# Christopher-Wang/DistriFlow

Measured on AMD Instinct MI355X. Metric: images/sec (whole node), MNIST CNN sync-SGD at 1/2/4/8 MI355X; async speedup, higher is better.
Workload: dtype bf16; 1 GPU; model=lenet5, global_batch=4096, per_gpu_batch=4096, parallelism=dp1, optimizer=sgd, graph=full, steps_per_graph=64, p2p_reason=single rank, step=train+reduce/update, params=61706

## Files before the change

csrc/bindings_fused.cpp:

```cpp
#include "bindings_comm.h"

namespace dfa_py {
namespace {

struct CPIn {
  const void* x = nullptr;
  int u8 = 0;
  const long long* idx = nullptr;
  long long nrows = 0;
};

CPIn cp_input(const torch::Tensor& x, const c10::optional<torch::Tensor>& idx, int64_t B, int64_t HWC) {
  CPIn r;
  TORCH_CHECK(x.is_cuda() && x.is_contiguous(), "x must be a contiguous GPU tensor");
  if (has(idx)) {
    need(*idx, at::kLong, "idx");
    TORCH_CHECK(idx->numel() >= B, "idx shorter than the batch");
    TORCH_CHECK(x.scalar_type() == at::kByte || x.scalar_type() == at::kBFloat16, "dataset must be u8 or bf16");
    TORCH_CHECK(x.dim() >= 1 && x.size(0) > 0 && x.numel() / x.size(0) == HWC, "dataset row size mismatch");
    TORCH_CHECK(x.scalar_type() == at::kByte, "indexed input must be a uint8 dataset");
    r.u8 = 1;
    r.idx = reinterpret_cast<const long long*>(idx->data_ptr<int64_t>());
    r.nrows = x.size(0);
  } else {
// ... 294 lines not shown

void lenet_train_py(torch::Tensor x, c10::optional<torch::Tensor> idx, double scale, torch::Tensor labels,
                    std::vector<torch::Tensor> conv, std::vector<torch::Tensor> dense_w,
                    std::vector<torch::Tensor> dense_wt, std::vector<torch::Tensor> dense_b,
                    std::vector<torch::Tensor> conv_grads, std::vector<torch::Tensor> dense_gw,
                    std::vector<torch::Tensor> dense_gb, std::vector<torch::Tensor> hT, std::vector<torch::Tensor> dzT,
                    torch::Tensor conv_part, torch::Tensor dense_part, torch::Tensor loss_part, torch::Tensor stats,
                    torch::Tensor frag, torch::Tensor ftab, torch::Tensor pxtab, int64_t B, double grad_scale,
                    bool prep, c10::optional<torch::Tensor> snap, std::vector<torch::Tensor> conv_mom,
                    c10::optional<torch::Tensor> sgd_master, c10::optional<torch::Tensor> sgd_mom,
                    c10::optional<torch::Tensor> sgd_wbf, c10::optional<torch::Tensor> sgd_hyper,
                    c10::optional<torch::Tensor> sgd_descs, c10::optional<torch::Tensor> idx_stream,
                    c10::optional<torch::Tensor> idx_cursor, c10::optional<torch::Tensor> idx_dst,
                    const P2PComm* ll, int64_t exch_blocks, c10::optional<torch::Tensor> run_stats,
                    const PSComm* ps, c10::optional<torch::Tensor> ps_perm, c10::optional<torch::Tensor> ps_idx,
                    double ps_lr, int64_t ps_max_stale, bool red_succ) {
  TORCH_CHECK(conv.size() == 4 && conv_grads.size() == 4, "lenet: conv = [w1, b1, w2, b2]");
  TORCH_CHECK(dense_w.size() == 3 && dense_wt.size() == 3 && dense_b.size() == 3 && dense_gw.size() == 3 &&
                  dense_gb.size() == 3 && hT.size() == 3 && dzT.size() == 3,
              "lenet: three dense layers");
  TORCH_CHECK(B > 0 && B < (1 << 30), "lenet: bad batch");
  dfa::LeNetArgs a{};
  const int64_t ldt = (B + 31) / 32 * 32;
  const int64_t lds = hT.size() == 3 && hT[0].dim() == 2 ? hT[0].size(1) : 0;
  TORCH_CHECK(lds >= ldt && lds % 32 == 0, "lenet: hT rows must hold round32(B) columns, stride a multiple of 32");
  if (x.scalar_type() == at::kByte) {
    TORCH_CHECK(x.is_cuda() && x.is_contiguous() && x.numel() % 784 == 0, "lenet: uint8 dataset [N][28][28][1]");
    a.x_u8 = x.data_ptr<uint8_t>();
    a.nrows = x.numel() / 784;
    TORCH_CHECK(has(idx) || a.nrows >= B,
                "lenet: a uint8 dataset without batch indices must hold the batch (rows 0 .. B-1)");
// ... 63 lines not shown
  a.loss_part = loss_part.data_ptr<float>();
  auto bp = [](torch::Tensor& t) { return reinterpret_cast<dfa::bf16*>(t.data_ptr()); };
  a.h0T = bp(hT[0]); a.h1T = bp(hT[1]); a.h2T = bp(hT[2]);
  a.dz1T = bp(dzT[0]); a.dz2T = bp(dzT[1]); a.dz3T = bp(dzT[2]);
  TORCH_CHECK(frag.is_cuda() && frag.is_contiguous() && (size_t)frag.nbytes() >= dfa::lenet_frag_bytes(),
              "lenet: fragment buffer too small");
  TORCH_CHECK(ftab.is_cuda() && ftab.scalar_type() == at::kByte && ftab.numel() == 98 * 2 * 16, "lenet: ftab");
  TORCH_CHECK(pxtab.is_cuda() && pxtab.scalar_type() == at::kShort && pxtab.numel() == 832, "lenet: pxtab");
  a.frag = frag.data_ptr();
  a.prep = prep ? 1 : 0;
  a.ftab = ftab.data_ptr<uint8_t>();
  a.pxtab = reinterpret_cast<const unsigned short*>(pxtab.data_ptr());
  a.B = (int)B;
  a.ldt = (int)lds;
  a.grad_scale = (float)grad_scale;
  dfa::LeNetRedArgs r{};
  r.kcols = (int)ldt;
  need(dense_part, at::kFloat, "lenet dense_part");
  TORCH_CHECK(dense_part.numel() >= dfa::lenet_dense_part_floats((int)B),
              "lenet: dense_part must hold lenet_dense_part_floats(B) zero-initialised floats");
  dfa::lenet_red_bind_scratch(dense_part.data_ptr<float>(), r);
  r.succ = red_succ ? 1 : 0;
  r.conv_part = a.conv_part;
  r.loss_part = a.loss_part;
  r.stats = stats.data_ptr<float>();
  r.g_w1 = conv_grads[0].data_ptr<float>();
  r.g_b1 = conv_grads[1].data_ptr<float>();
  r.g_w2 = conv_grads[2].data_ptr<float>();
  r.g_b2 = conv_grads[3].data_ptr<float>();
  for (int l = 0; l < 3; ++l) {
// ... 220 lines not shown
        py::arg("x"), py::arg("idx"), py::arg("scale"), py::arg("B"), py::arg("w1"), py::arg("b1"), py::arg("kpad1"),
        py::arg("w2t"), py::arg("dyp"), py::arg("code"), py::arg("slabs"), py::arg("g_w1"), py::arg("g_b1"),
        py::arg("g_w2"), py::arg("g_b2"), py::arg("step_inc") = py::none());
  m.def("kcnn_slab_floats", [](int64_t B) { return (int64_t)dfa::kcnn_slab_floats((int)B); });
  m.def("lenet_train", &lenet_train_py, "whole-network LeNet-5 training step (fwd + CE + bwd, 2 launches)",
        py::arg("x"), py::arg("idx"), py::arg("scale"), py::arg("labels"), py::arg("conv"), py::arg("dense_w"),
        py::arg("dense_wt"), py::arg("dense_b"), py::arg("conv_grads"), py::arg("dense_gw"), py::arg("dense_gb"),
        py::arg("hT"), py::arg("dzT"), py::arg("conv_part"), py::arg("dense_part"), py::arg("loss_part"),
        py::arg("stats"), py::arg("frag"), py::arg("ftab"), py::arg("pxtab"), py::arg("B"), py::arg("grad_scale"),
        py::arg("prep") = true, py::arg("snap") = py::none(),
        py::arg("conv_mom") = std::vector<torch::Tensor>{}, py::arg("sgd_master") = py::none(),
        py::arg("sgd_mom") = py::none(), py::arg("sgd_wbf") = py::none(), py::arg("sgd_hyper") = py::none(),
        py::arg("sgd_descs") = py::none(), py::arg("idx_stream") = py::none(), py::arg("idx_cursor") = py::none(),
        py::arg("idx_dst") = py::none(), py::arg("ll") = nullptr, py::arg("exch_blocks") = 0, py::arg("run_stats") = py::none(),
        py::arg("ps") = nullptr, py::arg("ps_perm") = py::none(), py::arg("ps_idx") = py::none(),
        py::arg("ps_lr") = 0.0, py::arg("ps_max_stale") = -1, py::arg("red_succ") = true);
  m.def("lenet_blocks", [](int64_t B) { return dfa::lenet_blocks((int)B); });
  m.def("lenet_frag_bytes", []() { return (int64_t)dfa::lenet_frag_bytes(); });
  m.def("lenet_dense_part_floats", [](int64_t B) { return (int64_t)dfa::lenet_dense_part_floats((int)B); });
  m.def("lenet_red_err_offset", []() { return (int64_t)dfa::lenet_red_err_offset(); });
}

void bind_comm(py::module_& m) {
  py::class_<P2PComm>(m, "P2PComm", "one-shot xGMI all-reduce over IPC-mapped peer buffers")
      .def(py::init<int64_t, int64_t, int64_t, double, int64_t>(), py::arg("rank"), py::arg("world"),
           py::arg("max_floats"), py::arg("timeout_s") = 2.0, py::arg("ll_slots") = 256)
      .def("handle", &P2PComm::handle)
      .def("open", &P2PComm::open)
      .def("allreduce", &P2PComm::allreduce, py::arg("t"), py::arg("scale") = 1.0)
      .def("error", &P2PComm::error)
      .def("host_error", &P2PComm::host_error)
      .def("ll_selftest", &P2PComm::ll_selftest, py::arg("inp"), py::arg("out"))
// ... 56 lines not shown
```

csrc/kernels.h:

```cpp
#pragma once
#include <hip/hip_runtime_api.h>
#include <stddef.h>
#include <stdint.h>

#include "ps_layout.h"

namespace dfa {
typedef __bf16 bf16;
}

namespace dfa {

enum { MODE_DIRECT = 0, MODE_FWD = 1, MODE_DGRAD = 2 };

struct DropSpec {
  int on;
  unsigned thresh;
  float p, scale;
  unsigned long long seed;
  const long long* step;
  int step_add;
};
inline DropSpec make_drop(float p, unsigned long long seed, const long long* step, int step_add = 0) {
  DropSpec d{};
// ... 398 lines not shown
  float* conv_part;
  float* loss_part;
  bf16 *h0T, *h1T, *h2T;
  bf16 *dz1T, *dz2T, *dz3T;
  float* logits;
  int prep;
  const void* frag;
  const unsigned char* ftab;
  const unsigned short* pxtab;
  unsigned long long* stamps;
  int B, ldt;
  float grad_scale;
  int nblk, ps_admit;
  int ps_excl;
  int ipw;
  PSArgs ps;
};
struct LeNetDense {
  const bf16* dzT;
  const bf16* hT;
  float* gw;
  float* gb;
  int N, K, tiles;
};
struct LeNetSgd {
  float* master;
  float* mom;
  bf16* wbf;
  const float* hyper;
  ParamDesc d[10];
// ... 106 lines not shown
  int ldt, jobs, nloss;
  const float* loss_part;
  float* stats;
};
hipError_t khead_wgrad(KHeadWgradArgs a, hipStream_t st);
size_t khead_ws_floats(int B, int K);
size_t khead_err_offset(int B);
size_t khead_lds(int K);
bool khead_supported(int K, int C);
hipError_t khead_train(KHeadArgs a, hipStream_t st);
int lenet_dense_part_floats(int B);
void lenet_red_bind_scratch(float* dense_part, LeNetRedArgs& r);
int lenet_red_err_offset();
size_t lenet_train_lds();
int lenet_blocks(int B);
hipError_t lenet_train(const LeNetArgs& a, LeNetRedArgs r, hipStream_t st);
void lenet_set_stamps(void* buf);
size_t lenet_frag_bytes();

enum MetricKind {
  kMetricMSE = 0, kMetricAbs = 1, kMetricHinge = 2, kMetricHuber = 3, kMetricLog = 4, kMetricSigmoidCE = 5,
  kMetricSoftmaxCE = 6, kMetricCategoricalCE = 7
};
hipError_t classifier_metrics(const float* z, const int* labels, int B, int C, int kind, int softmax, float* out,
                              hipStream_t st);

enum ActKind {
  kActLinear = 0, kActRelu = 1, kActRelu6 = 2, kActSigmoid = 3, kActTanh = 4, kActElu = 5, kActSelu = 6,
  kActSoftplus = 7, kActSoftsign = 8, kActHardSigmoid = 9, kActSwish = 10, kActExp = 11
};
// ... 36 lines not shown
```

csrc/lenet_fused.hip:

```cpp
#include "common.h"
#include "diag.h"
#include "kernels.h"
#include "lenet_frag.h"
#include "ll_exchange.h"
#include "optim_device.h"
#include "ps_device.h"

#include <algorithm>
#include <cstdlib>
#include <vector>

namespace dfa {
namespace {

constexpr int IMG = 8;
constexpr int NT = 512;
constexpr int NW = NT / 64;
constexpr int ccdiv(int a, int b) { return (a + b - 1) / b; }
constexpr int XS_ELEMS = IMG * 1024 + 32;
constexpr int OFF_XS = 0;
constexpr int OFF_P1 = OFF_XS + XS_ELEMS * 2;
constexpr int OFF_C1 = OFF_P1 + IMG * 196 * 16;
constexpr int DC2_RS = 104;
constexpr int NM = IMG * DC2_RS;
// ... 26 lines not shown
constexpr int LDS_BYTES = OFF_ST + 128;
static_assert(OFF_U == OFF_C1 + IMG * 196 * 4 + 128 + 98 * 2 * 16 + 800 * 2 + 128 && OFF_U % 16 == 0 && OFF_KZ % 16 == 0 && OFF_H1 % 16 == 0 && OFF_ZR % 16 == 0 && OFF_C2 % 16 == 0 && OFF_RED % 16 == 0 && OFF_DB % 16 == 0 && OFF_ST % 16 == 0 &&
                  OFF_PX % 16 == 0 && OFF_W % 16 == 0,
              "LDS carve must stay 16-byte aligned");
static_assert(2 * LDS_BYTES <= 160 * 1024, "two workgroups per CU");

typedef __bf16 bf16x4_vs __attribute__((__vector_size__(8)));

#define LN_STAMP(slot)                                                            \
  do {                                                                            \
    if (stamps) {                                                                 \
      __builtin_amdgcn_sched_barrier(0);                                          \
      unsigned long long t_;                                                      \
      asm volatile("s_memtime %0\n\ts_waitcnt lgkmcnt(0)" : "=s"(t_)::"memory"); \
      __builtin_amdgcn_sched_barrier(0);                                          \
      if (threadIdx.x == 0) STMP[(slot)] = t_;                                    \
    }                                                                             \
  } while (0)

template <int CTRL>
__device__ __forceinline__ float dpp_f(float v) {
  return __builtin_bit_cast(float, __builtin_amdgcn_update_dpp(0, __builtin_bit_cast(int, v), CTRL, 0xf, 0xf, false));
}
__device__ __forceinline__ float row16_max(float v) {
  v = fmaxf(v, dpp_f<0xB1>(v));
  v = fmaxf(v, dpp_f<0x4E>(v));
  v = fmaxf(v, dpp_f<0x141>(v));
  return fmaxf(v, dpp_f<0x140>(v));
}
__device__ __forceinline__ float row16_sum(float v) {
  v += dpp_f<0xB1>(v);
// ... 14 lines not shown
  for (int e = 0; e < 4; ++e) {
    r[e] = a[e];
    r[e + 4] = b[e];
  }
  return r;
}
__device__ __forceinline__ bf16x8 ld8(const bf16* p) { return *reinterpret_cast<const bf16x8*>(p); }
__device__ __forceinline__ void st8(bf16* p, const bf16x8& v) { *reinterpret_cast<bf16x8*>(p) = v; }
__device__ __forceinline__ bf16x8 zero8() {
  bf16x8 z;
#pragma unroll
  for (int e = 0; e < 8; ++e) z[e] = (bf16)0.f;
  return z;
}

__device__ __forceinline__ void build_shift1(const bf16* Xs, bf16* Xs1) {
  for (int t = threadIdx.x; t < XS_ELEMS / 8 - 1; t += NT) {
    const uint4 lo = *reinterpret_cast<const uint4*>(Xs + 8 * t);
    const unsigned nx = *reinterpret_cast<const unsigned*>(Xs + 8 * t + 8);
    uint4 o;
    o.x = __builtin_amdgcn_alignbyte(lo.y, lo.x, 2);
    o.y = __builtin_amdgcn_alignbyte(lo.z, lo.y, 2);
    o.z = __builtin_amdgcn_alignbyte(lo.w, lo.z, 2);
    o.w = __builtin_amdgcn_alignbyte(nx, lo.w, 2);
    *reinterpret_cast<uint4*>(Xs1 + 8 * t) = o;
  }
}

__device__ __forceinline__ void pool4(float a00, float a01, float a10, float a11, float& best, unsigned& code) {
  best = a00;
  code = 0;
  if (a01 > best) { best = a01; code = 1; }
  if (a10 > best) { best = a10; code = 2; }
  if (a11 > best) { best = a11; code = 3; }
  if (!(best > 0.f)) { best = 0.f; code = 4; }
}

template <int KS, int NTW>
struct DenseFrags {
  bf16x8 b[NTW][KS];
};
template <int KS, int NTW>
__device__ __forceinline__ void dense_load(DenseFrags<KS, NTW>& f, const bf16* __restrict__ W, int ntiles) {
  const int lane = threadIdx.x & 63, w = threadIdx.x >> 6, i = lane & 15, g = lane >> 4;
#pragma unroll
  for (int tt = 0; tt < NTW; ++tt) {
    const int t = w + NW * tt;
    if (t < ntiles) {
      const bf16* wrow = W + (long long)(16 * t + i) * (32 * KS) + 8 * g;
#pragma unroll
      for (int s = 0; s < KS; ++s) f.b[tt][s] = ld8(wrow + 32 * s);
    }
  }
}

template <int KS, int NTW>
__device__ __forceinline__ void dense_fwd(const DenseFrags<KS, NTW>& f, const bf16* A, int lda, const bf16* zr,
                                          const float* __restrict__ bias, int N, bool relu, bf16* out, int ldo,
                                          float* out32, bf16* __restrict__ hT, int ldt, int r0, int rows) {
  const int lane = threadIdx.x & 63, w = threadIdx.x >> 6, i = lane & 15, g = lane >> 4;
  const int ntiles = (N + 15) / 16;
  const bf16* arow = (i < IMG ? A + i * lda : zr) + 8 * g;
#pragma unroll
  for (int tt = 0; tt < NTW; ++tt) {
    const int t = w + NW * tt;
    if (t >= ntiles) break;
    const int n = 16 * t + i;
    f32x4 acc = {0.f, 0.f, 0.f, 0.f};
#pragma unroll
    for (int s = 0; s < KS; ++s) acc = mfma16x16x32(ld8(arow + 32 * s), f.b[tt][s], acc);
    if (g >= 2) continue;
    const float bv = (bias != nullptr && n < N) ? bias[n] : 0.f;
    float v[4];
#pragma unroll
    for (int r = 0; r < 4; ++r) {
      v[r] = acc[r] + bv;
      if (relu) v[r] = fmaxf(v[r], 0.f);
      if (n >= N) v[r] = 0.f;
      const int row = 4 * g + r;
      if (out) out[row * ldo + n] = f2bf(v[r]);
      if (out32) out32[row * 16 + (n & 15)] = v[r];
    }
    if (hT != nullptr && n < N) {
      bf16* dst = hT + (long long)n * ldt + r0 + 4 * g;
      if (4 * g + 4 <= rows) {
        bf16x4 pk;
#pragma unroll
        for (int r = 0; r < 4; ++r) pk[r] = f2bf(v[r]);
        *reinterpret_cast<bf16x4*>(dst) = pk;
      } else {
        for (int r = 0; r < 4; ++r)
          if (4 * g + r < rows) dst[r] = f2bf(v[r]);
      }
    }
  }
}

template <int KS, int NTW>
__device__ __forceinline__ void dense_bwd(const DenseFrags<KS, NTW>& f, const bf16* dZ, int ldz, const bf16* zr,
                                          int K, const bf16* mask, int ldm, bf16* out, int ldo,
                                          bf16* __restrict__ gT, int ldt, int r0, int rows) {
  const int lane = threadIdx.x & 63, w = threadIdx.x >> 6, i = lane & 15, g = lane >> 4;
  const int ktiles = (K + 15) / 16;
  const bf16* zrow = (i < IMG ? dZ + i * ldz : zr) + 8 * g;
#pragma unroll
  for (int tt = 0; tt < NTW; ++tt) {
    const int t = w + NW * tt;
    if (t >= ktiles) break;
    const int j = 16 * t + i;
    f32x4 acc = {0.f, 0.f, 0.f, 0.f};
#pragma unroll
    for (int s = 0; s < KS; ++s) acc = mfma16x16x32(ld8(zrow + 32 * s), f.b[tt][s], acc);
    if (g >= 2) continue;
    float v[4];
#pragma unroll
    for (int r = 0; r < 4; ++r) {
      const int row = 4 * g + r;
      v[r] = acc[r];
      if (mask != nullptr && !((float)mask[row * ldm + j] > 0.f)) v[r] = 0.f;
      if (j >= K) v[r] = 0.f;
      out[row * ldo + j] = f2bf(v[r]);
    }
    if (gT != nullptr && j < K) {
      bf16* dst = gT + (long long)j * ldt + r0 + 4 * g;
      if (4 * g + 4 <= rows) {
        bf16x4 pk;
#pragma unroll
        for (int r = 0; r < 4; ++r) pk[r] = f2bf(v[r]);
        *reinterpret_cast<bf16x4*>(dst) = pk;
      } else {
        for (int r = 0; r < 4; ++r)
          if (4 * g + r < rows) dst[r] = f2bf(v[r]);
      }
    }
  }
}

__device__ __forceinline__ int lenet_img_group(int b, int nb) {
  const int per = nb / 8;
  if (b >= 8 * per) return b;
  return (b & 7) * per + (b >> 3);
}

__device__ __forceinline__ void lenet_ps_owner_decide(const PSArgs& p, unsigned* s_cnt) {
  const int k = threadIdx.x;
  if (k < p.nshards) {
    const unsigned ep = __hip_atomic_load(p.scratch + kPSEpoch, __ATOMIC_RELAXED, __HIP_MEMORY_SCOPE_AGENT) + 1u;
// ... 27 lines not shown
__device__ __forceinline__ void lenet_ps_admission(const PSArgs& p, bool excl) {
  const long long bid = *p.bid_out;
  const unsigned applied0 = ps_read_applied(p);
  const unsigned ep = __hip_atomic_load(p.scratch + kPSEpoch, __ATOMIC_RELAXED, __HIP_MEMORY_SCOPE_AGENT) + 1u;
  const unsigned dec = ps_admit(p, false);
  const bool owner = p.owner_ring > 0;
  if (!owner && (dec == kPSAccept || dec == kPSReject)) ps_note_refresh(p, applied0 + (dec == kPSAccept ? 1u : 0u));
  __hip_atomic_store(p.scratch + kPSDecision, (ep << 3) | dec, __ATOMIC_RELAXED, __HIP_MEMORY_SCOPE_AGENT);
  if (excl) {
    __hip_atomic_store(p.scratch + kPSEpoch, ep, __ATOMIC_RELAXED, __HIP_MEMORY_SCOPE_AGENT);
    if (dec == kPSAccept) ps_publish_applied(p);
  }
  if (dec == kPSAccept && p.done_epoch != nullptr) complete_microbatch(p, bid);
}

template <bool TRIM>
__global__ void __launch_bounds__(NT, 2 * NT / 256) lenet_train_kernel(LeNetArgs a) {
  if ((int)blockIdx.x >= a.nblk) {
    if (a.ps_admit && threadIdx.x == 0) lenet_ps_admission(a.ps, a.ps_excl != 0);
    return;
  }
  extern __shared__ __attribute__((aligned(16))) char smem[];
  bf16* Xs = reinterpret_cast<bf16*>(smem + OFF_XS);
  bf16* Xs1 = reinterpret_cast<bf16*>(smem + OFF_XS1);
  bf16* P1 = reinterpret_cast<bf16*>(smem + OFF_P1);
  unsigned* C1 = reinterpret_cast<unsigned*>(smem + OFF_C1);
  bf16* KO = reinterpret_cast<bf16*>(smem + OFF_K);
  unsigned char* FT = reinterpret_cast<unsigned char*>(smem + OFF_FT);
  unsigned short* PX = reinterpret_cast<unsigned short*>(smem + OFF_PX);
  float* WS = reinterpret_cast<float*>(smem + OFF_W);
  bf16* H0 = reinterpret_cast<bf16*>(smem + OFF_H0);
  bf16* H1 = reinterpret_cast<bf16*>(smem + OFF_H1);
  bf16* H2 = reinterpret_cast<bf16*>(smem + OFF_H2);
  bf16* Z3 = reinterpret_cast<bf16*>(smem + OFF_Z3);
  bf16* Z2 = reinterpret_cast<bf16*>(smem + OFF_Z2);
  bf16* Z1 = reinterpret_cast<bf16*>(smem + OFF_Z1);
  bf16* ZR = reinterpret_cast<bf16*>(smem + OFF_ZR);
  float* LG = reinterpret_cast<float*>(smem + OFF_LG);
  unsigned char* C2 = reinterpret_cast<unsigned char*>(smem + OFF_C2);
  bf16* DC2 = reinterpret_cast<bf16*>(smem + OFF_DC2);
  float* RED = reinterpret_cast<float*>(smem + OFF_RED);

  const int tid = threadIdx.x, lane = tid & 63, w = __builtin_amdgcn_readfirstlane(tid >> 6), i = lane & 15,
            g = lane >> 4;
  const int r0 = lenet_img_group(blockIdx.x, a.nblk) * (TRIM ? a.ipw : IMG);
  const int rows = min(TRIM ? a.ipw : IMG, a.B - r0);
  const int nA = TRIM ? 2 * ((7 * rows + 1) / 2) : 56;
  const int nB = TRIM ? (13 * rows + 1) / 2 : NM / 16;
  const int nE = TRIM ? ((13 * rows + 3) / 4 + 1) / 2 * 2 : NM / 32;
  const int nF = TRIM ? (49 * rows + 7) / 8 : 49;
  const int nG = TRIM ? 14 * rows : IMG * 14;
  const bf16x8* __restrict__ frag = reinterpret_cast<const bf16x8*>(a.frag);
  float* part = a.conv_part + (long long)blockIdx.x * kLeNetConvStride;
  unsigned long long* const stamps = a.stamps;
  unsigned long long* const STMP = reinterpret_cast<unsigned long long*>(smem + OFF_ST);
  LN_STAMP(0);

  const int ximg = tid / 28, xrow = tid - 28 * (tid / 28);
  const bool xload = tid < IMG * 28 && ximg < rows;
  const bool lload = tid >= 256 && tid < 256 + IMG && tid - 256 < rows;
  long long xsrc = 0, lsrc = 0;
  if (xload) xsrc = a.idx ? a.idx[r0 + ximg] : (long long)(r0 + ximg);
  if (lload) lsrc = a.idx ? a.idx[r0 + tid - 256] : (long long)(r0 + tid - 256);
  uint4 tabv = {0u, 0u, 0u, 0u};
  if (tid < 98 * 2) tabv = reinterpret_cast<const uint4*>(a.ftab)[tid];
  else if (tid >= 264 && tid < 264 + NM / 8) tabv = reinterpret_cast<const uint4*>(a.pxtab)[tid - 264];
  static_assert(98 * 2 <= 256 && 264 + NM / 8 <= 448 && 448 + 22 <= NT, "phase 0 staging thread ranges");
  float biasv = 0.f, dbv = 0.f;
// ... 50 lines not shown
      for (int k = 0; k < 7; ++k)
#pragma unroll
        for (int h = 0; h < 2; ++h) {
          const float f0 = (float)((xv[k] >> (16 * h)) & 255u) * a.scale;
          const float f1 = (float)((xv[k] >> (16 * h + 8)) & 255u) * a.scale;
          const unsigned lo = __builtin_bit_cast(unsigned short, f2bf(f0));
          const unsigned hi = __builtin_bit_cast(unsigned short, f2bf(f1));
          dst[2 * k + h] = lo | (hi << 16);
        }
    } else {
#pragma unroll
      for (int k = 0; k < 14; ++k) dst[k] = xv[k];
    }
  }
  __syncthreads();
  build_shift1(Xs, Xs1);
  __syncthreads();
  LN_STAMP(1);

  {
    const float b1c[3] = {WS[(i >> 3)], WS[2 + (i >> 3)], WS[4 + (i >> 3)]};
#pragma unroll 2
    for (int u = w; u < nA; u += NT / 64) {
      const int mt = u >> 1, x0 = (u & 1) * 16;
      const int m = 16 * mt + i;
      const int img = m / 56, rem = m - 56 * (m / 56);
      const bf16* abase = ((rem & 1) ? Xs1 : Xs) + img * 1024 + (rem >> 1) * 32 + x0 + 8 * g;
      f32x4 acc[3];
#pragma unroll
      for (int T = 0; T < 3; ++T) acc[T] = {0.f, 0.f, 0.f, 0.f};
#pragma unroll
// ... 13 lines not shown
        pool4(acc[T][0] + b1c[T], acc[T][1] + b1c[T], acc[T][2] + b1c[T], acc[T][3] + b1c[T], best, code);
        const int c = 2 * T + (i >> 3);
        if (px < 14) P1[((imgo * 14 + py) * 14 + px) * 8 + c] = f2bf(best);
        cw |= code << (3 * c);
      }
      cw |= __shfl_xor(cw, 8, 64);
      if (i < 8 && px < 14) C1[(imgo * 14 + py) * 14 + px] = cw;
    }
  }
  __syncthreads();
  LN_STAMP(2);

  bf16x8 bw[7];
#pragma unroll
  for (int s = 0; s < 7; ++s) bw[s] = frag[(FR_C2 + s) * 64 + lane];
  DenseFrags<13, ccdiv(8, NW)> f1;
  dense_load(f1, a.d1w, 8);
  {
    int toff[7];
#pragma unroll
    for (int s = 0; s < 7; ++s) {
      const int tap = 4 * s + g;
      toff[s] = tap < 25 ? ((tap / 5) * 14 + (tap - 5 * (tap / 5))) * 8 : 0;
    }
    const float b2 = WS[6 + i];
#pragma unroll 2
    for (int mt = w; mt < nB; mt += NT / 64) {
      const bf16* abase = P1 + (int)PX[16 * mt + i] * 8;
      f32x4 acc = {0.f, 0.f, 0.f, 0.f};
#pragma unroll
      for (int s = 0; s < 7; ++s) acc = mfma16x16x32(ld8(abase + toff[s]), bw[s], acc);
      const int m0 = 16 * mt + 4 * g;
// ... 9 lines not shown
  }
  __syncthreads();
  LN_STAMP(3);

  for (int k = tid; k < 400; k += NT) {
    bf16* dst = a.h0T + (long long)k * a.ldt + r0;
    if (rows == IMG) {
      bf16x8 v;
#pragma unroll
      for (int r = 0; r < IMG; ++r) v[r] = H0[r * LD0 + k];
      st8(dst, v);
    } else {
      for (int r = 0; r < rows; ++r) dst[r] = H0[r * LD0 + k];
    }
  }
  DenseFrags<4, ccdiv(6, NW)> f2;
  DenseFrags<3, 1> f3;
  dense_load(f2, a.d2w, 6);
  dense_load(f3, a.d3w, 1);
  dense_fwd(f1, H0, LD0, ZR, DB, 120, true, H1, LD1, nullptr, a.h1T, a.ldt, r0, rows);
  __syncthreads();
  DenseFrags<1, ccdiv(6, NW)> g3;
  DenseFrags<3, ccdiv(8, NW)> g2;
  dense_load(g3, a.d3wt, 6);
  dense_load(g2, a.d2wt, 8);
  dense_fwd(f2, H1, LD1, ZR, DB + 120, 84, true, H2, LD2, nullptr, a.h2T, a.ldt, r0, rows);
  __syncthreads();
  dense_fwd(f3, H2, LD2, ZR, DB + 204, 10, false, nullptr, 0, LG, nullptr, a.ldt, r0, rows);
  __syncthreads();
  LN_STAMP(4);
  if (tid < IMG * 16) {
    const int r = tid >> 4, c = tid & 15;
    const bool live = r < rows;
    const int y = min(max(LBL[r], 0), 9);
    const float z = c < 10 ? LG[r * 16 + c] : -INFINITY;
    if (a.logits && live && c < 10) a.logits[(long long)(r0 + r) * 10 + c] = z;
    const float mx = row16_max(z);
    const unsigned long long hit = __ballot(z == mx);
    const int am = __builtin_ctzll((hit >> (16 * (r & 3))) | 0x10000ull);
    const float e = c < 10 ? __expf(z - mx) : 0.f;
    const float ssum = row16_sum(e);
    if (live && c < 10) {
      const float gv = (e * (1.f / ssum) - (c == y ? 1.f : 0.f)) * a.grad_scale;
      Z3[r * LD3 + c] = f2bf(gv);
      a.dz3T[(long long)c * a.ldt + r0 + r] = f2bf(gv);
    }
    if (c == y) LG[r * 16 + 14] = live ? -(z - mx - __logf(ssum)) : 0.f;
    if (c == 15) LG[r * 16 + 15] = (live && am == y) ? 1.f : 0.f;
  }
  __syncthreads();
  if (tid == 0) {
    float ls = 0.f, cs = 0.f;
#pragma unroll
    for (int r = 0; r < IMG; ++r) {
      ls += LG[r * 16 + 14];
      cs += LG[r * 16 + 15];
    }
    a.loss_part[2 * blockIdx.x] = ls;
    a.loss_part[2 * blockIdx.x + 1] = cs;
  }
  DenseFrags<4, ccdiv(25, NW)> g1;
  dense_load(g1, a.d1wt, 25);
  __syncthreads();
  LN_STAMP(5);
  dense_bwd(g3, Z3, LD3, ZR, 84, H2, LD2, Z2, LD2, a.dz2T, a.ldt, r0, rows);
  __syncthreads();
  dense_bwd(g2, Z2, LD2, ZR, 120, H1, LD1, Z1, LD1, a.dz1T, a.ldt, r0, rows);
  __syncthreads();
  dense_bwd(g1, Z1, LD1, ZR, 400, H0, LD0, H0, LD0, nullptr, 0, r0, rows);
  __syncthreads();
  LN_STAMP(6);

  {
    bf16x8 dp[2];
    unsigned long long cd[2];
#pragma unroll
    for (int k = 0; k < 2; ++k) {
      const int it = tid + k * NT;
      if (it < IMG * 50) {
        const int img = it / 50, rem = it - 50 * (it / 50), win = rem >> 1, nh = rem & 1;
        dp[k] = ld8(H0 + img * LD0 + win * 16 + 8 * nh);
        cd[k] = *reinterpret_cast<const unsigned long long*>(C2 + (img * 25 + win) * 16 + 8 * nh);
      }
    }
// ... 62 lines not shown
      const bf16x8 avb = ldAv(s + 1);
      const unsigned pxb0 = pxl[32 * (s + 1)], pxb1 = pxl[32 * (s + 1) + 4];
      __builtin_amdgcn_sched_barrier(0);
      step(ava, pxa0, pxa1);
      __builtin_amdgcn_sched_barrier(0);
      const int sn = s + 2 < nE ? s + 2 : s;
      ava = ldAv(sn);
      pxa0 = pxl[32 * sn];
      pxa1 = pxl[32 * sn + 4];
      __builtin_amdgcn_sched_barrier(0);
      step(avb, pxb0, pxb1);
      __builtin_amdgcn_sched_barrier(0);
    }
#pragma unroll
    for (int k = 0; k < KT; ++k) {
      if (k < ntile) {
        const int T = w + NW * k;
        const int tap = 2 * T + (i >> 3), c = i & 7;
#pragma unroll
        for (int r = 0; r < 4; ++r) {
          const int n = 4 * g + r;
          if (tap < 25 && c < 6) part[(long long)(kLeNetPW2 + n * 150 + tap * 6 + c)] = acc[k][r];
          else if (tap == 0 && c == 6) part[(long long)(kLeNetPB2 + n)] = acc[k][r];
        }
      }
    }
  }
  __syncthreads();
  LN_STAMP(8);

  {
// ... 16 lines not shown
        acc = mfma16x16x32(a0, bd[s], acc);
        a0 = a1;
        a1 = a2;
        if (s + 3 < 15) a2 = ldA(s + 3);
      }
      if (c < 6) {
#pragma unroll
        for (int r = 0; r < 4; ++r) {
          const int mm = 16 * mt + 4 * g + r;
          P1[(2 * mm + bcol) * 8 + c] = f2bf(acc[r]);
        }
      }
    }
  }
  __syncthreads();
  build_shift1(Xs, Xs1);
  __syncthreads();
  LN_STAMP(9);

  {
    f32x4 acc[2] = {{0.f, 0.f, 0.f, 0.f}, {0.f, 0.f, 0.f, 0.f}};
    const int gdy = i >= 6 && i < 12 ? 1 : 0;
    const int ca = i < 6 ? i : (i < 12 ? i - 6 : 5);
    constexpr int kXs1 = (OFF_XS1 - OFF_XS) / 2;
    unsigned boff[2], bconst[2];
    bool breal[2];
#pragma unroll
    for (int T = 0; T < 2; ++T) {
      const int e = 16 * T + i;
      const int ep = e < 30 ? e : 0;
      const int ky = ep / 5, kx = ep - 5 * (ep / 5);
// ... 36 lines not shown
    __syncthreads();
    if (w < 4) {
#pragma unroll
      for (int T = 0; T < 2; ++T)
#pragma unroll
        for (int r = 0; r < 4; ++r) {
          float* q = RED + (w * 16 + 4 * g + r) * 32 + 16 * T + i;
          *q = (NW > 4 ? *q : 0.f) + acc[T][r];
        }
    }
    __syncthreads();
    auto S = [&](int row, int col) {
      return RED[(0 * 16 + row) * 32 + col] + RED[(1 * 16 + row) * 32 + col] + RED[(2 * 16 + row) * 32 + col] +
             RED[(3 * 16 + row) * 32 + col];
    };
    for (int e = tid; e < 6 * 26; e += NT) {
      const int c = e / 26, t = e - 26 * (e / 26);
      if (t < 25) part[(long long)(kLeNetPW1 + c * 25 + t)] = S(c, t) + S(6 + c, t + 5);
      else part[(long long)(kLeNetPB1 + c)] = S(c, 30) + S(6 + c, 30);
    }
  }
  LN_STAMP(10);
  if (stamps && tid < 11) stamps[blockIdx.x * 16 + tid] = STMP[tid];
}

constexpr int PT = 1024;
__global__ void __launch_bounds__(PT) lenet_prep_kernel(const float* __restrict__ w1g, const float* __restrict__ w2g,
                                                        bf16x8* __restrict__ frag) {
  __shared__ float w[kLeNetConvW];
  for (int e = threadIdx.x; e < 150; e += PT) w[e] = w1g[e];
  for (int e = threadIdx.x; e < 2400; e += PT) w[150 + e] = w2g[e];
  __syncthreads();
  lenet_build_frags(w, frag, threadIdx.x, PT);
}

constexpr int RT = 256;
constexpr int kDU = 32;
constexpr int kChunks = 8;
// ... 987 lines not shown
}

size_t lenet_train_lds() { return LDS_BYTES; }
int lenet_ipw(int B) {
  static const int forced = diag_int("lenet_ipw", 0);
  if (forced == 1 || forced == 2 || forced == 4 || forced == IMG) return forced;
  int ipw = 1;
  while (ipw < IMG && (B + ipw - 1) / ipw > 256) ipw *= 2;
  return ipw;
}
int lenet_blocks(int B) {
  const int ipw = lenet_ipw(B);
  return (B + ipw - 1) / ipw;
}

static unsigned long long* g_lenet_stamps_host = nullptr;
void lenet_set_stamps(void* buf) { g_lenet_stamps_host = reinterpret_cast<unsigned long long*>(buf); }

size_t lenet_frag_bytes() { return (size_t)NFRAG * 64 * 16; }

static int lenet_red_slots() {
  const int NK[3][2] = {{120, 400}, {84, 120}, {10, 84}};
  int n = (kLeNetConvParams + kConvPer - 1) / kConvPer;
  for (auto& nk : NK) n += ((nk[0] + kDU - 1) / kDU) * ((nk[1] + 1 + kDU - 1) / kDU);
  return n;
}
static int lenet_red_slab_floats() { return lenet_red_slots() * kChunks * kSlotVals; }
static int lenet_red_ep_words() { return (kChunks * (lenet_red_slots() + 1) + 3) / 4 * 4; }
int lenet_dense_part_floats(int B) {
  (void)B;
// ... 91 lines not shown
        r.ps.shard_shift < 6 || ((r.ps.n - 1) >> r.ps.shard_shift) >= r.ps.nshards)
      return hipErrorInvalidValue;
    for (int k = 0; k < r.ps.nshards; ++k)
      if (!r.ps.shard[k]) return hipErrorInvalidValue;
    if (r.ps.owner_ring > 0) {
      if (r.ps.owner_ring > 255 || r.ps.max_stale < 0 || r.ps.owner_ring < r.ps.max_stale + 2 || !r.ps.pref ||
          !r.ps.dlock || r.ps.rank < 0)
        return hipErrorInvalidValue;
      for (int k = 0; k < r.ps.nshards; ++k)
        if (!r.ps.inbox[k]) return hipErrorInvalidValue;
    }
  }
  const bool psx = r.ps_on && r.ps.excl != 0 && r.succ && r.ps.nshards == 1 && r.ps.owner_ring <= 0;
  a.ps_excl = psx ? 1 : 0;
  r.mirror = psx ? r.ps.shard[0] : nullptr;
  if (a.ipw < IMG)
    hipLaunchKernelGGL(lenet_train_kernel<true>, dim3(nblk + (r.ps_on ? 1 : 0)), dim3(NT), LDS_BYTES, st, a);
  else
    hipLaunchKernelGGL(lenet_train_kernel<false>, dim3(nblk + (r.ps_on ? 1 : 0)), dim3(NT), LDS_BYTES, st, a);
  DFA_HIP_CHECK(hipGetLastError());
  const int extra = r.ps_on ? 2 : ((r.sgd_on && r.sgd.src) ? 1 : 0);
  const dim3 grid(r.exch_blocks + 1 + extra);
  if (r.ll_on) hipLaunchKernelGGL(lenet_reduce_kernel<1>, grid, dim3(RT), 0, st, r);
  else if (psx) hipLaunchKernelGGL(lenet_reduce_kernel<3>, grid, dim3(RT), 0, st, r);
  else if (r.ps_on && r.ps.owner_ring > 0) hipLaunchKernelGGL(lenet_reduce_kernel<4>, grid, dim3(RT), 0, st, r);
  else if (r.ps_on) hipLaunchKernelGGL(lenet_reduce_kernel<2>, grid, dim3(RT), 0, st, r);
  else hipLaunchKernelGGL(lenet_reduce_kernel<0>, grid, dim3(RT), 0, st, r);
  return hipGetLastError();
}

}
```

distriflow_amd/diagnostics.py:

```python
from __future__ import annotations

import os

_DEFAULTS = {"lenet_fused": 1, "lenet_fused_update": 1, "async_fused": 1, "ps_owner_apply": -1, "ps_excl_fused": 1, "kcnn_fused": 1, "khead_fused": 1, "fold_dropout": 1,
             "lenet_succ": 1, "multistep": 1, "graph_steps": 64, "fused_selftest": 1, "wgrad_overlap": 0, "proj_overlap": 0, "concurrent_backward": 0,
             "bn_acc": 1, "bn_acc_rep": 8}


def diag(name: str) -> int:
    if name not in _DEFAULTS:
        raise KeyError(f"unknown diagnostic switch {name!r}")
    spec = os.environ.get("DISTRIFLOW_DIAG", "")
    for item in spec.split(","):
        k, _, v = item.strip().partition("=")
        if k == name and v:
            return int(v)
    return _DEFAULTS[name]


def on(name: str) -> bool:
    return diag(name) != 0


def active() -> dict:
# ... 2 lines not shown
```

distriflow_amd/ops/__init__.py:

```python
from __future__ import annotations

import torch

from .. import native
from ..diagnostics import on as _diag_on
from . import reference as ref

MODE_DIRECT, MODE_FWD, MODE_DGRAD = 0, 1, 2


class _DebugSync:

    def __init__(self, mod):
        self._mod = mod

    def __getattr__(self, name):
        fn = getattr(self._mod, name)
        if not callable(fn) or isinstance(fn, type):
            return fn

        def wrapped(*args, **kw):
            out = fn(*args, **kw)
            if torch.cuda.is_available() and not torch.cuda.is_current_stream_capturing():
                try:
# ... 732 lines not shown


def lenet_supported() -> bool:
    m = native.get(build_if_missing=False)
    return m is not None and hasattr(m, "lenet_train")


def lenet_frag_bytes() -> int:
    return int(_C().lenet_frag_bytes())


def lenet_blocks(B: int) -> int:
    return int(_C().lenet_blocks(int(B)))


_LENET_TABLES = {}


def lenet_tables(device):
    key = str(device)
    if key not in _LENET_TABLES:
        import numpy as np

        swz = lambda t: t ^ ((t >> 3) & 7)
        ft = np.full((98, 2, 16), swz(100), dtype=np.uint8)
        for yx in range(98):
            y, X2 = divmod(yx, 7)
            for hf in range(2):
                for s in range(16):
                    P = 2 * s + hf
# ... 28 lines not shown
        src, idx, scale = x.data, x.idx, x.scale
    else:
        src, idx, scale = x.contiguous(), None, 1.0
    if isinstance(labels, LabelRef):
        lab, lidx = labels.labels, labels.idx
        if idx is None:
            idx = lidx
    else:
        lab = labels if labels.dtype == torch.int32 else labels.to(torch.int32)
    B = x.shape[0]
    ftab, pxtab, scratch = lenet_tables(stats.device)
    _C().lenet_train(src, idx, float(scale), lab, list(conv), list(dense_w), list(dense_wt), list(dense_b),
                     list(conv_grads), list(dense_gw), list(dense_gb), list(hT), list(dzT), conv_part, dense_part,
                     loss_part, stats, scratch if frag is None else frag, ftab, pxtab, int(B), float(grad_scale),
                     prep=bool(prep) or frag is None, snap=snap, conv_mom=list(conv_mom),
                     red_succ=_diag_on("lenet_succ"), **(sgd or {}))


def lenet_red_error(dense_part) -> int:
    o = int(_C().lenet_red_err_offset())
    return int(dense_part[o:o + 1].view(torch.int32)[0].item())


def convpool_supported(H, W, C, KH, KW, pad, N) -> bool:
    m = native.get(build_if_missing=False)
    if m is None:
        return False
    return bool(m.convpool_supported(H, W, C, KH, KW, pad, N))


def convpool_fwd_layout(H, W, C, KH, KW, pad, N):
# ... 71 lines not shown
```

Measured before the change: 71.43 million images/s.

## Pair two 8-image LeNet blocks per workgroup to fill 16-row MFMA tiles

Adds a paired variant of the fused LeNet-5 train kernel in which one double-size workgroup processes two 8-image blocks, each half with its own LDS region. In the dense forward and backward layers the two halves' activations feed the 16 rows of each MFMA tile, so the half of every tile that previously carried zero padding now does useful work and each wave handles half as many dense tiles. The variant is chosen automatically for large untrimmed batches when neither the parameter-server nor the P2P path is active. The cost is a larger workgroup with double LDS, changed launch bounds that may alter register allocation and occupancy, an earlier load of the first-layer backward weights, and extra guards for a half with no blocks assigned.

Result: no change. 71.95 million images/s (median of 6 runs) (+0.7%).

```diff
diff --git a/csrc/bindings_fused.cpp b/csrc/bindings_fused.cpp
--- a/csrc/bindings_fused.cpp
+++ b/csrc/bindings_fused.cpp
@@ -332,7 +332,7 @@
                     c10::optional<torch::Tensor> idx_cursor, c10::optional<torch::Tensor> idx_dst,
                     const P2PComm* ll, int64_t exch_blocks, c10::optional<torch::Tensor> run_stats,
                     const PSComm* ps, c10::optional<torch::Tensor> ps_perm, c10::optional<torch::Tensor> ps_idx,
-                    double ps_lr, int64_t ps_max_stale, bool red_succ) {
+                    double ps_lr, int64_t ps_max_stale, bool red_succ, int64_t lenet_pair) {
   TORCH_CHECK(conv.size() == 4 && conv_grads.size() == 4, "lenet: conv = [w1, b1, w2, b2]");
   TORCH_CHECK(dense_w.size() == 3 && dense_wt.size() == 3 && dense_b.size() == 3 && dense_gw.size() == 3 &&
                   dense_gb.size() == 3 && hT.size() == 3 && dzT.size() == 3,
@@ -426,6 +426,7 @@
   a.B = (int)B;
   a.ldt = (int)lds;
   a.grad_scale = (float)grad_scale;
+  a.pair = lenet_pair < 0 ? -1 : (lenet_pair > 0 ? 1 : 0);
   dfa::LeNetRedArgs r{};
   r.kcols = (int)ldt;
   need(dense_part, at::kFloat, "lenet dense_part");
@@ -676,8 +677,12 @@
         py::arg("sgd_descs") = py::none(), py::arg("idx_stream") = py::none(), py::arg("idx_cursor") = py::none(),
         py::arg("idx_dst") = py::none(), py::arg("ll") = nullptr, py::arg("exch_blocks") = 0, py::arg("run_stats") = py::none(),
         py::arg("ps") = nullptr, py::arg("ps_perm") = py::none(), py::arg("ps_idx") = py::none(),
-        py::arg("ps_lr") = 0.0, py::arg("ps_max_stale") = -1, py::arg("red_succ") = true);
+        py::arg("ps_lr") = 0.0, py::arg("ps_max_stale") = -1, py::arg("red_succ") = true,
+        py::arg("lenet_pair") = -1);
   m.def("lenet_blocks", [](int64_t B) { return dfa::lenet_blocks((int)B); });
+  m.def("lenet_paired", [](int64_t B, int64_t pair) {
+    return dfa::lenet_paired((int)B, (int)pair);
+  }, "whether a batch of B runs the paired LeNet-5 train kernel under switch value pair (-1 auto, 0, 1)");
   m.def("lenet_frag_bytes", []() { return (int64_t)dfa::lenet_frag_bytes(); });
   m.def("lenet_dense_part_floats", [](int64_t B) { return (int64_t)dfa::lenet_dense_part_floats((int)B); });
   m.def("lenet_red_err_offset", []() { return (int64_t)dfa::lenet_red_err_offset(); });
diff --git a/csrc/kernels.h b/csrc/kernels.h
--- a/csrc/kernels.h
+++ b/csrc/kernels.h
@@ -436,6 +436,7 @@
   int nblk, ps_admit;
   int ps_excl;
   int ipw;
+  int pair;
   PSArgs ps;
 };
 struct LeNetDense {
@@ -572,6 +573,7 @@
 int lenet_red_err_offset();
 size_t lenet_train_lds();
 int lenet_blocks(int B);
+bool lenet_paired(int B, int pair);
 hipError_t lenet_train(const LeNetArgs& a, LeNetRedArgs r, hipStream_t st);
 void lenet_set_stamps(void* buf);
 size_t lenet_frag_bytes();
diff --git a/csrc/lenet_fused.hip b/csrc/lenet_fused.hip
--- a/csrc/lenet_fused.hip
+++ b/csrc/lenet_fused.hip
@@ -64,7 +64,7 @@
       unsigned long long t_;                                                      \
       asm volatile("s_memtime %0\n\ts_waitcnt lgkmcnt(0)" : "=s"(t_)::"memory"); \
       __builtin_amdgcn_sched_barrier(0);                                          \
-      if (threadIdx.x == 0) STMP[(slot)] = t_;                                    \
+      if (tid == 0) STMP[(slot)] = t_;                                            \
     }                                                                             \
   } while (0)
 
@@ -109,8 +109,8 @@
   return z;
 }
 
-__device__ __forceinline__ void build_shift1(const bf16* Xs, bf16* Xs1) {
-  for (int t = threadIdx.x; t < XS_ELEMS / 8 - 1; t += NT) {
+__device__ __forceinline__ void build_shift1(const bf16* Xs, bf16* Xs1, int tid) {
+  for (int t = tid; t < XS_ELEMS / 8 - 1; t += NT) {
     const uint4 lo = *reinterpret_cast<const uint4*>(Xs + 8 * t);
     const unsigned nx = *reinterpret_cast<const unsigned*>(Xs + 8 * t + 8);
     uint4 o;
@@ -135,12 +135,12 @@
 struct DenseFrags {
   bf16x8 b[NTW][KS];
 };
-template <int KS, int NTW>
+template <int NWD, int KS, int NTW>
 __device__ __forceinline__ void dense_load(DenseFrags<KS, NTW>& f, const bf16* __restrict__ W, int ntiles) {
   const int lane = threadIdx.x & 63, w = threadIdx.x >> 6, i = lane & 15, g = lane >> 4;
 #pragma unroll
   for (int tt = 0; tt < NTW; ++tt) {
-    const int t = w + NW * tt;
+    const int t = w + NWD * tt;
     if (t < ntiles) {
       const bf16* wrow = W + (long long)(16 * t + i) * (32 * KS) + 8 * g;
 #pragma unroll
@@ -149,22 +149,32 @@
   }
 }
 
-template <int KS, int NTW>
+constexpr int HALF_ELEMS = LDS_BYTES / 2;
+struct DenseRows {
+  int r0[2], rows[2];
+};
+
+template <int NWD, int KS, int NTW>
 __device__ __forceinline__ void dense_fwd(const DenseFrags<KS, NTW>& f, const bf16* A, int lda, const bf16* zr,
                                           const float* __restrict__ bias, int N, bool relu, bf16* out, int ldo,
-                                          float* out32, bf16* __restrict__ hT, int ldt, int r0, int rows) {
+                                          float* out32, bf16* __restrict__ hT, int ldt, const DenseRows& dr) {
+  constexpr bool PAIR = NWD > NW;
   const int lane = threadIdx.x & 63, w = threadIdx.x >> 6, i = lane & 15, g = lane >> 4;
   const int ntiles = (N + 15) / 16;
-  const bf16* arow = (i < IMG ? A + i * lda : zr) + 8 * g;
+  const bf16* arow = (PAIR ? A + (i >> 3) * HALF_ELEMS + (i & 7) * lda : (i < IMG ? A + i * lda : zr)) + 8 * g;
+  const int hh = PAIR ? g >> 1 : 0, gl = PAIR ? g & 1 : g;
+  const int r0 = hh ? dr.r0[1] : dr.r0[0], rows = hh ? dr.rows[1] : dr.rows[0];
+  if (PAIR && out) out += hh * HALF_ELEMS;
+  if (PAIR && out32) out32 += hh * (HALF_ELEMS / 2);
 #pragma unroll
   for (int tt = 0; tt < NTW; ++tt) {
-    const int t = w + NW * tt;
+    const int t = w + NWD * tt;
     if (t >= ntiles) break;
     const int n = 16 * t + i;
     f32x4 acc = {0.f, 0.f, 0.f, 0.f};
 #pragma unroll
     for (int s = 0; s < KS; ++s) acc = mfma16x16x32(ld8(arow + 32 * s), f.b[tt][s], acc);
-    if (g >= 2) continue;
+    if (!PAIR && g >= 2) continue;
     const float bv = (bias != nullptr && n < N) ? bias[n] : 0.f;
     float v[4];
 #pragma unroll
@@ -172,60 +182,65 @@
       v[r] = acc[r] + bv;
       if (relu) v[r] = fmaxf(v[r], 0.f);
       if (n >= N) v[r] = 0.f;
-      const int row = 4 * g + r;
+      const int row = 4 * gl + r;
       if (out) out[row * ldo + n] = f2bf(v[r]);
       if (out32) out32[row * 16 + (n & 15)] = v[r];
     }
     if (hT != nullptr && n < N) {
-      bf16* dst = hT + (long long)n * ldt + r0 + 4 * g;
-      if (4 * g + 4 <= rows) {
+      bf16* dst = hT + (long long)n * ldt + r0 + 4 * gl;
+      if (4 * gl + 4 <= rows) {
         bf16x4 pk;
 #pragma unroll
         for (int r = 0; r < 4; ++r) pk[r] = f2bf(v[r]);
         *reinterpret_cast<bf16x4*>(dst) = pk;
       } else {
         for (int r = 0; r < 4; ++r)
-          if (4 * g + r < rows) dst[r] = f2bf(v[r]);
-      }
-    }
-  }
-}
-
-template <int KS, int NTW>
+          if (4 * gl + r < rows) dst[r] = f2bf(v[r]);
+      }
+    }
+  }
+}
+
+template <int NWD, int KS, int NTW>
 __device__ __forceinline__ void dense_bwd(const DenseFrags<KS, NTW>& f, const bf16* dZ, int ldz, const bf16* zr,
                                           int K, const bf16* mask, int ldm, bf16* out, int ldo,
-                                          bf16* __restrict__ gT, int ldt, int r0, int rows) {
+                                          bf16* __restrict__ gT, int ldt, const DenseRows& dr) {
+  constexpr bool PAIR = NWD > NW;
   const int lane = threadIdx.x & 63, w = threadIdx.x >> 6, i = lane & 15, g = lane >> 4;
   const int ktiles = (K + 15) / 16;
-  const bf16* zrow = (i < IMG ? dZ + i * ldz : zr) + 8 * g;
+  const bf16* zrow = (PAIR ? dZ + (i >> 3) * HALF_ELEMS + (i & 7) * ldz : (i < IMG ? dZ + i * ldz : zr)) + 8 * g;
+  const int hh = PAIR ? g >> 1 : 0, gl = PAIR ? g & 1 : g;
+  const int r0 = hh ? dr.r0[1] : dr.r0[0], rows = hh ? dr.rows[1] : dr.rows[0];
+  if (PAIR) out += hh * HALF_ELEMS;
+  if (PAIR && mask) mask += hh * HALF_ELEMS;
 #pragma unroll
   for (int tt = 0; tt < NTW; ++tt) {
-    const int t = w + NW * tt;
+    const int t = w + NWD * tt;
     if (t >= ktiles) break;
     const int j = 16 * t + i;
     f32x4 acc = {0.f, 0.f, 0.f, 0.f};
 #pragma unroll
     for (int s = 0; s < KS; ++s) acc = mfma16x16x32(ld8(zrow + 32 * s), f.b[tt][s], acc);
-    if (g >= 2) continue;
+    if (!PAIR && g >= 2) continue;
     float v[4];
 #pragma unroll
     for (int r = 0; r < 4; ++r) {
-      const int row = 4 * g + r;
+      const int row = 4 * gl + r;
       v[r] = acc[r];
       if (mask != nullptr && !((float)mask[row * ldm + j] > 0.f)) v[r] = 0.f;
       if (j >= K) v[r] = 0.f;
       out[row * ldo + j] = f2bf(v[r]);
     }
     if (gT != nullptr && j < K) {
-      bf16* dst = gT + (long long)j * ldt + r0 + 4 * g;
-      if (4 * g + 4 <= rows) {
+      bf16* dst = gT + (long long)j * ldt + r0 + 4 * gl;
+      if (4 * gl + 4 <= rows) {
         bf16x4 pk;
 #pragma unroll
         for (int r = 0; r < 4; ++r) pk[r] = f2bf(v[r]);
         *reinterpret_cast<bf16x4*>(dst) = pk;
       } else {
         for (int r = 0; r < 4; ++r)
-          if (4 * g + r < rows) dst[r] = f2bf(v[r]);
+          if (4 * gl + r < rows) dst[r] = f2bf(v[r]);
       }
     }
   }
@@ -283,13 +298,21 @@
   if (dec == kPSAccept && p.done_epoch != nullptr) complete_microbatch(p, bid);
 }
 
-template <bool TRIM>
-__global__ void __launch_bounds__(NT, 2 * NT / 256) lenet_train_kernel(LeNetArgs a) {
-  if ((int)blockIdx.x >= a.nblk) {
+constexpr int lenet_pairs(int nblk) { return (nblk >> 4) * 8 + ((nblk & 15) < 8 ? (nblk & 15) : 8); }
+
+template <bool TRIM, bool PAIR>
+__global__ void __launch_bounds__(PAIR ? 2 * NT : NT, 4) lenet_train_kernel(LeNetArgs a) {
+  static_assert(!(TRIM && PAIR), "a paired workgroup holds full 8-image blocks");
+  if ((int)blockIdx.x >= (PAIR ? lenet_pairs(a.nblk) : a.nblk)) {
     if (a.ps_admit && threadIdx.x == 0) lenet_ps_admission(a.ps, a.ps_excl != 0);
     return;
   }
-  extern __shared__ __attribute__((aligned(16))) char smem[];
+  extern __shared__ __attribute__((aligned(16))) char smem0[];
+  const int wv = __builtin_amdgcn_readfirstlane((int)threadIdx.x >> 6);
+  const int hf = PAIR ? wv >> 3 : 0;
+  char* const smem = smem0 + hf * LDS_BYTES;
+  const int b = PAIR ? ((int)blockIdx.x >> 3) * 16 + ((int)blockIdx.x & 7) + 8 * hf : (int)blockIdx.x;
+  const bool hlive = !PAIR || b < a.nblk;
   bf16* Xs = reinterpret_cast<bf16*>(smem + OFF_XS);
   bf16* Xs1 = reinterpret_cast<bf16*>(smem + OFF_XS1);
   bf16* P1 = reinterpret_cast<bf16*>(smem + OFF_P1);
@@ -310,17 +333,25 @@
   bf16* DC2 = reinterpret_cast<bf16*>(smem + OFF_DC2);
   float* RED = reinterpret_cast<float*>(smem + OFF_RED);
 
-  const int tid = threadIdx.x, lane = tid & 63, w = __builtin_amdgcn_readfirstlane(tid >> 6), i = lane & 15,
-            g = lane >> 4;
-  const int r0 = lenet_img_group(blockIdx.x, a.nblk) * (TRIM ? a.ipw : IMG);
-  const int rows = min(TRIM ? a.ipw : IMG, a.B - r0);
+  const int tid = PAIR ? (int)threadIdx.x & (NT - 1) : (int)threadIdx.x, lane = tid & 63, w = PAIR ? wv & 7 : wv,
+            i = lane & 15, g = lane >> 4;
+  const int r0 = hlive ? lenet_img_group(b, a.nblk) * (TRIM ? a.ipw : IMG) : 0;
+  const int rows = hlive ? min(TRIM ? a.ipw : IMG, a.B - r0) : 0;
+  DenseRows dr = {{r0, 0}, {rows, 0}};
+  if (PAIR) {
+    const int b0 = b - 8 * hf, b1 = b0 + 8;
+    dr.r0[0] = lenet_img_group(b0, a.nblk) * IMG;
+    dr.rows[0] = min(IMG, a.B - dr.r0[0]);
+    dr.r0[1] = b1 < a.nblk ? lenet_img_group(b1, a.nblk) * IMG : 0;
+    dr.rows[1] = b1 < a.nblk ? min(IMG, a.B - dr.r0[1]) : 0;
+  }
   const int nA = TRIM ? 2 * ((7 * rows + 1) / 2) : 56;
   const int nB = TRIM ? (13 * rows + 1) / 2 : NM / 16;
   const int nE = TRIM ? ((13 * rows + 3) / 4 + 1) / 2 * 2 : NM / 32;
   const int nF = TRIM ? (49 * rows + 7) / 8 : 49;
   const int nG = TRIM ? 14 * rows : IMG * 14;
   const bf16x8* __restrict__ frag = reinterpret_cast<const bf16x8*>(a.frag);
-  float* part = a.conv_part + (long long)blockIdx.x * kLeNetConvStride;
+  float* part = a.conv_part + (long long)b * kLeNetConvStride;
   unsigned long long* const stamps = a.stamps;
   unsigned long long* const STMP = reinterpret_cast<unsigned long long*>(smem + OFF_ST);
   LN_STAMP(0);
@@ -401,7 +432,7 @@
     }
   }
   __syncthreads();
-  build_shift1(Xs, Xs1);
+  build_shift1(Xs, Xs1, tid);
   __syncthreads();
   LN_STAMP(1);
 
@@ -445,8 +476,9 @@
   bf16x8 bw[7];
 #pragma unroll
   for (int s = 0; s < 7; ++s) bw[s] = frag[(FR_C2 + s) * 64 + lane];
-  DenseFrags<13, ccdiv(8, NW)> f1;
-  dense_load(f1, a.d1w, 8);
+  constexpr int NWD = PAIR ? 2 * NW : NW;
+  DenseFrags<13, ccdiv(8, NWD)> f1;
+  dense_load<NWD>(f1, a.d1w, 8);
   {
     int toff[7];
 #pragma unroll
@@ -486,19 +518,30 @@
       for (int r = 0; r < rows; ++r) dst[r] = H0[r * LD0 + k];
     }
   }
-  DenseFrags<4, ccdiv(6, NW)> f2;
+  char* const dsm = PAIR ? smem0 : smem;
+  bf16* const dH0 = reinterpret_cast<bf16*>(dsm + OFF_H0);
+  bf16* const dH1 = reinterpret_cast<bf16*>(dsm + OFF_H1);
+  bf16* const dH2 = reinterpret_cast<bf16*>(dsm + OFF_H2);
+  bf16* const dZ3 = reinterpret_cast<bf16*>(dsm + OFF_Z3);
+  bf16* const dZ2 = reinterpret_cast<bf16*>(dsm + OFF_Z2);
+  bf16* const dZ1 = reinterpret_cast<bf16*>(dsm + OFF_Z1);
+  float* const dLG = reinterpret_cast<float*>(dsm + OFF_LG);
+  const float* const dDB = reinterpret_cast<const float*>(dsm + OFF_DB);
+  DenseFrags<4, ccdiv(6, NWD)> f2;
   DenseFrags<3, 1> f3;
-  dense_load(f2, a.d2w, 6);
-  dense_load(f3, a.d3w, 1);
-  dense_fwd(f1, H0, LD0, ZR, DB, 120, true, H1, LD1, nullptr, a.h1T, a.ldt, r0, rows);
-  __syncthreads();
-  DenseFrags<1, ccdiv(6, NW)> g3;
-  DenseFrags<3, ccdiv(8, NW)> g2;
-  dense_load(g3, a.d3wt, 6);
-  dense_load(g2, a.d2wt, 8);
-  dense_fwd(f2, H1, LD1, ZR, DB + 120, 84, true, H2, LD2, nullptr, a.h2T, a.ldt, r0, rows);
-  __syncthreads();
-  dense_fwd(f3, H2, LD2, ZR, DB + 204, 10, false, nullptr, 0, LG, nullptr, a.ldt, r0, rows);
+  dense_load<NWD>(f2, a.d2w, 6);
+  dense_load<NWD>(f3, a.d3w, 1);
+  dense_fwd<NWD>(f1, dH0, LD0, ZR, dDB, 120, true, dH1, LD1, nullptr, a.h1T, a.ldt, dr);
+  __syncthreads();
+  DenseFrags<1, ccdiv(6, NWD)> g3;
+  DenseFrags<3, ccdiv(8, NWD)> g2;
+  dense_load<NWD>(g3, a.d3wt, 6);
+  dense_load<NWD>(g2, a.d2wt, 8);
+  DenseFrags<4, ccdiv(25, NWD)> g1;
+  if (PAIR) dense_load<NWD>(g1, a.d1wt, 25);
+  dense_fwd<NWD>(f2, dH1, LD1, ZR, dDB + 120, 84, true, dH2, LD2, nullptr, a.h2T, a.ldt, dr);
+  __syncthreads();
+  dense_fwd<NWD>(f3, dH2, LD2, ZR, dDB + 204, 10, false, nullptr, 0, dLG, nullptr, a.ldt, dr);
   __syncthreads();
   LN_STAMP(4);
   if (tid < IMG * 16) {
@@ -521,25 +564,24 @@
     if (c == 15) LG[r * 16 + 15] = (live && am == y) ? 1.f : 0.f;
   }
   __syncthreads();
-  if (tid == 0) {
+  if (tid == 0 && hlive) {
     float ls = 0.f, cs = 0.f;
 #pragma unroll
     for (int r = 0; r < IMG; ++r) {
       ls += LG[r * 16 + 14];
       cs += LG[r * 16 + 15];
     }
-    a.loss_part[2 * blockIdx.x] = ls;
-    a.loss_part[2 * blockIdx.x + 1] = cs;
-  }
-  DenseFrags<4, ccdiv(25, NW)> g1;
-  dense_load(g1, a.d1wt, 25);
+    a.loss_part[2 * b] = ls;
+    a.loss_part[2 * b + 1] = cs;
+  }
+  if (!PAIR) dense_load<NWD>(g1, a.d1wt, 25);
   __syncthreads();
   LN_STAMP(5);
-  dense_bwd(g3, Z3, LD3, ZR, 84, H2, LD2, Z2, LD2, a.dz2T, a.ldt, r0, rows);
-  __syncthreads();
-  dense_bwd(g2, Z2, LD2, ZR, 120, H1, LD1, Z1, LD1, a.dz1T, a.ldt, r0, rows);
-  __syncthreads();
-  dense_bwd(g1, Z1, LD1, ZR, 400, H0, LD0, H0, LD0, nullptr, 0, r0, rows);
+  dense_bwd<NWD>(g3, dZ3, LD3, ZR, 84, dH2, LD2, dZ2, LD2, a.dz2T, a.ldt, dr);
+  __syncthreads();
+  dense_bwd<NWD>(g2, dZ2, LD2, ZR, 120, dH1, LD1, dZ1, LD1, a.dz1T, a.ldt, dr);
+  __syncthreads();
+  dense_bwd<NWD>(g1, dZ1, LD1, ZR, 400, dH0, LD0, dH0, LD0, nullptr, 0, dr);
   __syncthreads();
   LN_STAMP(6);
 
@@ -632,7 +674,7 @@
     }
 #pragma unroll
     for (int k = 0; k < KT; ++k) {
-      if (k < ntile) {
+      if (k < ntile && hlive) {
         const int T = w + NW * k;
         const int tap = 2 * T + (i >> 3), c = i & 7;
 #pragma unroll
@@ -679,7 +721,7 @@
     }
   }
   __syncthreads();
-  build_shift1(Xs, Xs1);
+  build_shift1(Xs, Xs1, tid);
   __syncthreads();
   LN_STAMP(9);
 
@@ -746,14 +788,14 @@
       return RED[(0 * 16 + row) * 32 + col] + RED[(1 * 16 + row) * 32 + col] + RED[(2 * 16 + row) * 32 + col] +
              RED[(3 * 16 + row) * 32 + col];
     };
-    for (int e = tid; e < 6 * 26; e += NT) {
+    for (int e = tid; e < (hlive ? 6 * 26 : 0); e += NT) {
       const int c = e / 26, t = e - 26 * (e / 26);
       if (t < 25) part[(long long)(kLeNetPW1 + c * 25 + t)] = S(c, t) + S(6 + c, t + 5);
       else part[(long long)(kLeNetPB1 + c)] = S(c, 30) + S(6 + c, 30);
     }
   }
   LN_STAMP(10);
-  if (stamps && tid < 11) stamps[blockIdx.x * 16 + tid] = STMP[tid];
+  if (stamps && hlive && tid < 11) stamps[b * 16 + tid] = STMP[tid];
 }
 
 constexpr int PT = 1024;
@@ -1771,6 +1813,11 @@
   return (B + ipw - 1) / ipw;
 }
 
+bool lenet_paired(int B, int pair) {
+  const int nblk = lenet_blocks(B);
+  return lenet_ipw(B) == IMG && (pair > 0 || (pair < 0 && nblk >= 512 && lenet_pairs(nblk) <= 256));
+}
+
 static unsigned long long* g_lenet_stamps_host = nullptr;
 void lenet_set_stamps(void* buf) { g_lenet_stamps_host = reinterpret_cast<unsigned long long*>(buf); }
 
@@ -1892,10 +1939,14 @@
   const bool psx = r.ps_on && r.ps.excl != 0 && r.succ && r.ps.nshards == 1 && r.ps.owner_ring <= 0;
   a.ps_excl = psx ? 1 : 0;
   r.mirror = psx ? r.ps.shard[0] : nullptr;
-  if (a.ipw < IMG)
-    hipLaunchKernelGGL(lenet_train_kernel<true>, dim3(nblk + (r.ps_on ? 1 : 0)), dim3(NT), LDS_BYTES, st, a);
-  else
-    hipLaunchKernelGGL(lenet_train_kernel<false>, dim3(nblk + (r.ps_on ? 1 : 0)), dim3(NT), LDS_BYTES, st, a);
+  if (a.ipw < IMG) {
+    hipLaunchKernelGGL((lenet_train_kernel<true, false>), dim3(nblk + (r.ps_on ? 1 : 0)), dim3(NT), LDS_BYTES, st, a);
+  } else if (a.pair > 0 || (a.pair < 0 && !r.ps_on && !r.ll_on && lenet_paired(a.B, -1))) {
+    hipLaunchKernelGGL((lenet_train_kernel<false, true>), dim3(lenet_pairs(nblk) + (r.ps_on ? 1 : 0)), dim3(2 * NT),
+                       2 * LDS_BYTES, st, a);
+  } else {
+    hipLaunchKernelGGL((lenet_train_kernel<false, false>), dim3(nblk + (r.ps_on ? 1 : 0)), dim3(NT), LDS_BYTES, st, a);
+  }
   DFA_HIP_CHECK(hipGetLastError());
   const int extra = r.ps_on ? 2 : ((r.sgd_on && r.sgd.src) ? 1 : 0);
   const dim3 grid(r.exch_blocks + 1 + extra);
diff --git a/distriflow_amd/diagnostics.py b/distriflow_amd/diagnostics.py
--- a/distriflow_amd/diagnostics.py
+++ b/distriflow_amd/diagnostics.py
@@ -3,7 +3,7 @@
 import os
 
 _DEFAULTS = {"lenet_fused": 1, "lenet_fused_update": 1, "async_fused": 1, "ps_owner_apply": -1, "ps_excl_fused": 1, "kcnn_fused": 1, "khead_fused": 1, "fold_dropout": 1,
-             "lenet_succ": 1, "multistep": 1, "graph_steps": 64, "fused_selftest": 1, "wgrad_overlap": 0, "proj_overlap": 0, "concurrent_backward": 0,
+             "lenet_succ": 1, "lenet_pair": -1, "multistep": 1, "graph_steps": 64, "fused_selftest": 1, "wgrad_overlap": 0, "proj_overlap": 0, "concurrent_backward": 0,
              "bn_acc": 1, "bn_acc_rep": 8}
 
 
diff --git a/distriflow_amd/ops/__init__.py b/distriflow_amd/ops/__init__.py
--- a/distriflow_amd/ops/__init__.py
+++ b/distriflow_amd/ops/__init__.py
@@ -3,6 +3,7 @@
 import torch
 
 from .. import native
+from ..diagnostics import diag as _diag
 from ..diagnostics import on as _diag_on
 from . import reference as ref
 
@@ -770,6 +771,10 @@
     return int(_C().lenet_blocks(int(B)))
 
 
+def lenet_paired(B: int, pair: int | None = None) -> bool:
+    return bool(_C().lenet_paired(int(B), int(_diag("lenet_pair") if pair is None else pair)))
+
+
 _LENET_TABLES = {}
 
 
@@ -828,7 +833,7 @@
                      list(conv_grads), list(dense_gw), list(dense_gb), list(hT), list(dzT), conv_part, dense_part,
                      loss_part, stats, scratch if frag is None else frag, ftab, pxtab, int(B), float(grad_scale),
                      prep=bool(prep) or frag is None, snap=snap, conv_mom=list(conv_mom),
-                     red_succ=_diag_on("lenet_succ"), **(sgd or {}))
+                     red_succ=_diag_on("lenet_succ"), lenet_pair=_diag("lenet_pair"), **(sgd or {}))
 
 
 def lenet_red_error(dense_part) -> int:
```
